# pswpswpsw/nif

Hardware: AMD Instinct MI355X
Metric: train-step points/sec (1D-wave, batch=1M per GPU) (higher is better)
Workload: dtype f32

## Files before the change

nif_amd/csrc/k_snet6.hip:

```cpp
#include "k_fuse_dev.h"

#define ZERO_T6(x) _Pragma("unroll") for (int b_ = 0; b_ < NBL; ++b_) { (x)[b_][0] = 0.f; (x)[b_][1] = 0.f; (x)[b_][2] = 0.f; (x)[b_][3] = 0.f; }

template <int NBL>
__device__ __forceinline__ void ring_store16(float* __restrict__ slot, const f32x4 (&h)[NBL], int g, int p) {
  float* q = slot + 4 * g * 16 + p;
#pragma unroll
  for (int b = 0; b < NBL; ++b)
#pragma unroll
    for (int v = 0; v < 4; ++v) q[(16 * b + v) * 16] = h[b][v];
}
template <int NBL>
__device__ __forceinline__ void ring_load16(const float* __restrict__ slot, f32x4 (&h)[NBL], int g, int p) {
  const float* q = slot + 4 * g * 16 + p;
#pragma unroll
  for (int b = 0; b < NBL; ++b)
#pragma unroll
    for (int v = 0; v < 4; ++v) h[b][v] = q[(16 * b + v) * 16];
}

#ifdef NIF_TIMELINE
#define S6_TL(id) do { if (blockIdx.x == 0 && (tid == 0 || tid == 512) && tlr == 2 && tlc < 380) { tlb[tlc] = ((long long)(id) << 48) | ((long long)__builtin_amdgcn_s_memtime() & 0xFFFFFFFFFFFFll); ++tlc; } } while (0)
#define S6_TL_FLUSH() do { if (A.tl && blockIdx.x == 0 && (tid == 0 || tid == 512)) for (int q_ = 0; q_ < tlc; ++q_) { A.tl[(tid ? 2048 : 0) + 2 * q_] = tlb[q_] >> 48; A.tl[(tid ? 2048 : 0) + 2 * q_ + 1] = tlb[q_] & 0xFFFFFFFFFFFFll; } } while (0)
#else
#define S6_TL(id) do { } while (0)
#define S6_TL_FLUSH() do { } while (0)
#endif
struct S6Args {
  SNetArgs s;
  float* partial; long pstride;
};

#ifndef NIF_S6_DBAR_T0
#define NIF_S6_DBAR_T0 5
#endif

constexpr int S6_WAVES = 8, S6_MAX_WG = 256;
constexpr int s6_ring(int NBL) { return 16 * NBL * 16; }

template <int NBL, int PR = 0>
__global__ __launch_bounds__(1024, 4) void k_snet6(S6Args F) {
  extern __shared__ __attribute__((aligned(256))) char smem6[];
  const SNetArgs& A = F.s;
  constexpr int NT = 512, WAVES = S6_WAVES, r = 1;
  constexpr int NCH = NBL / 2;
  constexpr bool X16 = PR == 0;
  constexpr int CF = X16 ? NBL * 2 * 64 : NBL * 3 * 64, CB = NBL * 2 * 64;
  constexpr bool CP = PR != 0;
  constexpr int CFH = CP ? NBL * 64 : CF, CBH = CP ? NBL * 64 : CB;
  constexpr PlaneSet HSET = CP ? PLANES_COMPACT : PLANES_HALF;
  static_assert(CFH == plane_chunk_units(HSET, PLANE_FWD, NBL) && CBH == plane_chunk_units(HSET, PLANE_BWD, NBL), "k_pack_dev.h");
  constexpr bool BIG = X16;
  constexpr int CFB = BIG ? 2 * CF : CF;
  constexpr int QF = (CFB + NT - 1) / NT;
  constexpr int NBUF = 2;
  constexpr int NPL = 6;
  constexpr int EXT = NPL * FUSE_PLANE_BYTES;
  constexpr int NVL = 5, NVF = 8, WVLT = NVL * 64, WVFT = NVF * 64;
  const int tid = threadIdx.x, wid = __builtin_amdgcn_readfirstlane(tid >> 6);
  const int lane = tid & 63, p = lane & 15, g = lane >> 4;
  const int n = A.n, nh = A.nh, si = A.si, so = A.so;
  const long nt16 = 2 * ((A.B + 31) / 32);
  const long ngroups = (nt16 + WAVES - 1) / WAVES;

  char* EX = smem6;
  char* WVL = EX + WAVES * EXT;
  char* WVF = WVL + WAVES * WVLT;
  bf16x8* chunks = reinterpret_cast<bf16x8*>(WVF + WAVES * WVFT);
  float* sm = reinterpret_cast<float*>(chunks + NBUF * CFB);
  constexpr int NP = 16 * NBL, RING = s6_ring(NBL);
  constexpr int o_w1 = 0, o_wl = 3 * NP, o_b1 = 6 * NP, o_bh = 7 * NP, o_bl = 11 * NP, nsm = 11 * NP + 4;
  constexpr int sm_tot = ((r + 1) * nsm + 3) & ~3;
  constexpr int CX = 3, CZ = 1, CY = 3;
  constexpr int NI = (CX + CZ + CY + 1) * 16;
  constexpr int pw = 2 * r * 64 + 2 * NI;
  float* lsum = sm + sm_tot + (long)WAVES * pw;
  float* scl = lsum + 16;
  long long* tlb = reinterpret_cast<long long*>(scl + 16) + (tid ? 380 : 0); (void)tlb;

  {
    const long s_wl = (long)si * n + (long)nh * n * n;
    const long s_b1 = s_wl + (long)n * so, s_bh = s_b1 + n, s_bl = s_bh + (long)nh * n;
    for (int idx = tid; idx < (r + 1) * nsm; idx += 1024) {
      const int k = idx / nsm, e = idx - k * nsm;
      float v = 0.f;
      if (e < o_wl) { const int dd = e / NP, f = e - dd * NP; if (f < n && dd < si) v = A.omega * hyp3(A, k, (long)dd * n + f); }
      else if (e < o_b1) { const int o = (e - o_wl) / NP, f = (e - o_wl) - o * NP; if (f < n && o < so) v = hyp3(A, k, s_wl + (long)f * so + o); }
      else if (e < o_bh) { const int f = e - o_b1; if (f < n) v = hyp3(A, k, s_b1 + f); }
      else if (e < o_bl) {
        const int j = (e - o_bh) / NP, f = (e - o_bh) - j * NP;
        if (f < n && j < nh) {
          v = hyp3(A, k, s_bh + (long)j * n + f);
          if (X16) v *= 4096.0f * A.wscale[(j * (r + 1) + k) * 2];
        }
      }
      else if (e < o_bl + so) v = hyp3(A, k, s_bl + (e - o_bl));
      sm[idx] = v;
    }
    if (X16 && tid < nh * (r + 1) * 2) scl[tid] = A.wscale[tid];
    for (int idx = tid; idx < (WAVES * (EXT + WVLT + WVFT)) / 16; idx += 1024) reinterpret_cast<f32x4*>(EX)[idx] = f32x4{0.f, 0.f, 0.f, 0.f};
  }

  const int NPC = (r + 1) * NCH;
  const bf16x8* cs_src = reinterpret_cast<const bf16x8*>(A.WF4);
  const int NPCS = BIG ? (r + 1) : NPC;
  int cs_units = BIG ? 2 * CFH : CFH, cs_left = nh * NPCS, cs_phase = 0;
  long cs_groups = (ngroups - 1 - (long)blockIdx.x) / gridDim.x;
  auto cs_phase_step = [&]() {
    ++cs_phase;
    if (cs_phase < 1 + nh) {
// ... 233 lines not shown
    return;
  }
#undef bacc
#undef facc
#undef fbacc
#undef lacc
#undef blacc

  float* dzs = sm + sm_tot + (long)wid * pw;
  float* sks = dzs + r * 64;
  float* inp = sks + r * 64;
  auto prefetch_inputs = [&](long tgn, int set) {
    long t16n = tgn * WAVES + wid;
    if (t16n >= nt16) t16n = nt16 - 1;
    const long tile32n = t16n >> 1;
    const int poffn = 16 * (int)(t16n & 1) + p;
    long ptn = t16n * 16 + p;
    if (ptn >= A.B) ptn = A.B - 1;
    float* dst = inp + set * NI;
    {
      const int c = g < si ? g : si - 1;
      const float* src = g < 3 ? A.xin + ptn * A.ncol + A.col0 + c : A.Z + (tile32n * r) * 32 + poffn;
      __builtin_amdgcn_global_load_lds((const __attribute__((address_space(1))) void*)src,
                                       (__attribute__((address_space(3))) void*)dst, 4, 0, 0);
    }
    {
      const int c = g < so ? g : so - 1;
      const float* src = (g < 3 || !A.sw) ? A.y + ptn * so + c : A.sw + ptn;
      __builtin_amdgcn_global_load_lds((const __attribute__((address_space(1))) void*)src,
                                       (__attribute__((address_space(3))) void*)(dst + 4 * 16), 4, 0, 0);
    }
  };
  prefetch_inputs(blockIdx.x, 0);
  if (cs_left <= 0) cs_left = -1;
  cs_next(0, true);
  __syncthreads();
  bool dma_mine = false;
  bool dma_early = false;
  int cbuf = 0, nbuf = 1;
  int tlc = 0, tlr = 0; (void)tlc; (void)tlr;
  float loss_lane = 0.f;
  float* ring = A.stash + ((long)blockIdx.x * WAVES + wid) * (long)nh * RING;
  const FuseDep dep = fuse_dep_addr(p, g);
  char* exw = EX + wid * EXT;

#define S6_CHUNK(...)                                                         \
  {                                                                           \
    S6_TL(100);                                                               \
    if (!dma_early) cs_next(nbuf, dma_mine);                                  \
    dma_early = false;                                                        \
    S6_TL(200);                                                               \
    const bf16x8* cur = chunks + cbuf * CFB;                                  \
    __VA_ARGS__                                                               \
    S6_TL(300);                                                               \
    __builtin_amdgcn_s_waitcnt(0x0070);         \
    S6_TL(400);                                                               \
    asm volatile("" ::: "memory");                                            \
    __builtin_amdgcn_s_barrier();                                             \
    asm volatile("" ::: "memory");                                            \
    S6_TL(500);                                                               \
    cbuf ^= 1; nbuf ^= 1;                                                     \
  }
#define S6_CHUNK2(ZI_, Q0_, Q1_, T_)                                          \
  S6_CHUNK({ mfma_x3<NBL, 3, ZI_, NBL, 0, false>(cur, Q0_[0], Q1_[0], T_, lane); mfma_x3<NBL, 3, false, NBL, 0, false>(cur + CF, Q0_[1], Q1_[1], T_, lane); })

  int iset = 0;
  for (long tg = blockIdx.x; tg < ngroups; tg += gridDim.x, ++iset, ++tlr) {
    S6_TL(1);
    const long t16_raw = tg * WAVES + wid;
    const bool active = t16_raw < nt16;
    const long t16 = active ? t16_raw : nt16 - 1;
    const long tile32 = t16 >> 1;
    const int poff = 16 * (int)(t16 & 1) + p;
    const long pt = t16 * 16 + p;
    const bool valid = active && pt < A.B;
    const float* xs = inp + (iset & 1) * NI + p;
    const float* zs = inp + (iset & 1) * NI + CX * 16;
    const float* ys = zs + CZ * 16 + p;
    const float* wsp = zs + (CZ + CY) * 16 + p;
    const float* zt_base = zs + p;
    dzs[lane] = 0.f;

    f32x4 h[NBL], acc[NBL];
    auto first_layer = [&](f32x4 (&out)[NBL]) __attribute__((always_inline)) {
      f32x4 a_[NBL];
      {
        const float* s0 = sm + r * nsm + 4 * g;
#pragma unroll
        for (int b = 0; b < NBL; ++b) {
          f32x4 s = *reinterpret_cast<const f32x4*>(s0 + o_b1 + 16 * b);
          _Pragma("unroll") for (int dd = 0; dd < 3; ++dd) if (dd < si) s += xs[dd * 16] * *reinterpret_cast<const f32x4*>(s0 + o_w1 + dd * NP + 16 * b);
          a_[b] = s;
        }
      }
      {
        const float zt = zt_base[0];
        const float* s0 = sm + 4 * g;
#pragma unroll
        for (int b = 0; b < NBL; ++b) {
          f32x4 s = *reinterpret_cast<const f32x4*>(s0 + o_b1 + 16 * b);
          _Pragma("unroll") for (int dd = 0; dd < 3; ++dd) if (dd < si) s += xs[dd * 16] * *reinterpret_cast<const f32x4*>(s0 + o_w1 + dd * NP + 16 * b);
          a_[b] += zt * s;
        }
      }
      sine16_tag<NBL>(a_, out);
    };
    first_layer(h);
    prefetch_inputs(tg + gridDim.x, (iset + 1) & 1);
    dma_mine = false;
    for (int j = 0; j < nh; ++j) {
      bf16x8 b0[NCH], b1[NCH], b2[NCH];
      if (X16) split2h<NBL>(h, 4096.0f, b0, b1);
      else split3p<NBL, PR>(h, b0, b1, b2);
      const float s1_ = X16 ? scl[j * 4 + 2] : 1.0f, is0_ = X16 ? scl[j * 4 + 1] : 1.0f, is1_ = X16 ? scl[j * 4 + 3] : 1.0f;
      {
        const float* sb = sm + r * nsm + o_bh + j * NP + 4 * g;
#pragma unroll
        for (int b = 0; b < NBL; ++b) acc[b] = *reinterpret_cast<const f32x4*>(sb + 16 * b);
      }
      {
        f32x4 T[NBL];
        const float* sb = sm + o_bh + j * NP + 4 * g;
#pragma unroll
        for (int b = 0; b < NBL; ++b) T[b] = *reinterpret_cast<const f32x4*>(sb + 16 * b);
#define S6_FWD(KS_, T_) mfma_x6<NBL, PR, false, NBL, 0, CP>(cur, b0[KS_], b1[KS_], b2[KS_], T_, lane);
        if (j > 0) ring_store16<NBL>(ring + j * RING, h, g, p);
        if (BIG) S6_CHUNK2(false, b0, b1, T)
        else {
          S6_CHUNK(S6_FWD(0, T))
          S6_CHUNK(S6_FWD(1, T))
        }
        const float zt = X16 ? zt_base[0] * (s1_ * is0_) : zt_base[0];
#pragma unroll
        for (int b = 0; b < NBL; ++b) acc[b] += zt * T[b];
      }
      if (BIG) S6_CHUNK2(false, b0, b1, acc)
      else {
        S6_CHUNK(S6_FWD(0, acc))
        S6_CHUNK(S6_FWD(1, acc))
      }
#undef S6_FWD
      if (X16) sine16_tag_sc<NBL>(acc, acc, is1_ * (1.0f / 4096.0f));
      else sine16_tag<NBL>(acc, acc);
#pragma unroll
      for (int b = 0; b < NBL; ++b) h[b] = acc[b];
    }
    f32x4 gh[NBL];
    ZERO_T6(gh)
    const float wsamp = (valid ? (A.sw ? wsp[0] : 1.0f) : 0.0f);
    const float zt0 = zt_base[0];
    float se = 0.f;
    for (int o = 0; o < so; ++o) {
      f32x4 wg[NBL];
      ZERO_T6(wg)
      float part = 0.f, bias = 0.f;
#pragma unroll
      for (int k = 0; k <= r; ++k) {
        const float zt = k < r ? zt0 : 1.0f;
        const float* s0 = sm + k * nsm;
        float sk = 0.f, sk2 = 0.f;
#pragma unroll
        for (int b = 0; b < NBL; ++b) {
          const f32x4 w = *reinterpret_cast<const f32x4*>(s0 + o_wl + o * NP + 16 * b + 4 * g);
          sk = fmaf(h[b][0], w[0], sk); sk2 = fmaf(h[b][1], w[1], sk2); sk = fmaf(h[b][2], w[2], sk); sk2 = fmaf(h[b][3], w[3], sk2);
          wg[b] += zt * w;
        }
        sk += sk2;
        part = fmaf(zt, sk, part);
        bias = fmaf(zt, s0[o_bl + o], bias);
        if (k < r) sks[k * 64 + lane] = sk;
      }
      part += __shfl_xor(part, 16);
      part += __shfl_xor(part, 32);
      const float uo = part + bias;
      const float e = uo - ys[o * 16];
      NIF_LOSS_ACC(A.loss_kind, e, se, dfac)
      const float du = dfac * wsamp * A.inv_bg / (float)so;
#pragma unroll
      for (int b = 0; b < NBL; ++b) gh[b] += du * wg[b];
      {
        float t = du * sks[lane];
        if (g == 0) t = fmaf(du, sm[o_bl + o], t);
        dzs[lane] += t;
      }
      if (g == 0 && o < 3) {
        __bf16* wv = reinterpret_cast<__bf16*>(WVL + wid * WVLT);
        const __bf16 d0 = (__bf16)du;
        wv[o * 32 + p] = d0; wv[o * 32 + 16 + p] = (__bf16)(du - (float)d0);
      }
    }
    if (g == 1) {
      __bf16* wv = reinterpret_cast<__bf16*>(WVL + wid * WVLT);
      const __bf16 z0 = (__bf16)zt0;
      wv[3 * 32 + p] = z0; wv[3 * 32 + 16 + p] = (__bf16)(zt0 - (float)z0);
    }
    {
      bf16x8 a0[NCH], a1[NCH];
      split2<NBL>(h, a0, a1);
      fuse_deposit4(exw, dep, a0);
      fuse_deposit4(exw + FUSE_PLANE_BYTES, dep, a1);
      f32x4 zh[NBL];
#pragma unroll
      for (int b = 0; b < NBL; ++b) zh[b] = zt0 * h[b];
      split2<NBL>(zh, a0, a1);
      fuse_deposit4(exw + 2 * FUSE_PLANE_BYTES, dep, a0);
      fuse_deposit4(exw + 3 * FUSE_PLANE_BYTES, dep, a1);
    }
    if (g == 0) loss_lane += wsamp * se / (float)so * A.inv_bg;
    if (BIG) {
      asm volatile("" ::: "memory");
      __builtin_amdgcn_s_waitcnt(0xC07F);
      S6_TL(600);
      __builtin_amdgcn_s_barrier();
      asm volatile("" ::: "memory");
      S6_TL(700);
    }
    f32x4 dnext[NBL], hin[NBL];
#pragma unroll
    for (int b = 0; b < NBL; ++b) hin[b] = h[b];
    dma_mine = true;
    for (int j = nh - 1; j >= 0; --j) {
      f32x4 ga[NBL];
      if (BIG) { cs_next(nbuf, true); dma_early = true; }
      tag_cos<NBL>(hin, dnext);
#pragma unroll
      for (int b = 0; b < NBL; ++b) ga[b] = dnext[b] * gh[b];
      {
        const float* sb = sm + o_bh + j * NP + 4 * g;
        float sbv = 0.f, sbv2 = 0.f;
#pragma unroll
        for (int b = 0; b < NBL; ++b) {
          const f32x4 bb = *reinterpret_cast<const f32x4*>(sb + 16 * b);
          sbv = fmaf(ga[b][0], bb[0], sbv); sbv2 = fmaf(ga[b][1], bb[1], sbv2); sbv = fmaf(ga[b][2], bb[2], sbv); sbv2 = fmaf(ga[b][3], bb[3], sbv2);
        }
        sbv += sbv2;
        dzs[lane] += X16 ? sbv * (scl[j * 4 + 1] * (1.0f / 4096.0f)) : sbv;
      }
      bf16x8 b0[NCH], b1[NCH];
      split2<NBL>(ga, b0, b1);
      bf16x8 q0[NCH], q1[NCH];
      const float s1_ = X16 ? scl[j * 4 + 2] : 1.0f, is0_ = X16 ? scl[j * 4 + 1] : 1.0f, is1_ = X16 ? scl[j * 4 + 3] : 1.0f;
      float ils = 1.0f;
      if (PR == 2 || X16) {
        float mx = 0.f;
#pragma unroll
        for (int b = 0; b < NBL; ++b) mx = fmaxf(fmaxf(mx, fmaxf(fabsf(ga[b][0]), fabsf(ga[b][1]))), fmaxf(fabsf(ga[b][2]), fabsf(ga[b][3])));
        mx = fmaxf(mx, __shfl_xor(mx, 16));
        mx = fmaxf(mx, __shfl_xor(mx, 32));
        const unsigned ef = (__float_as_uint(mx) >> 23) & 0xFFu;
        const unsigned sf = 268u - ef < 227u ? 268u - ef : 227u;
        ils = __uint_as_float((254u - sf) << 23);
        if (X16) split2h<NBL>(ga, __uint_as_float(sf << 23), q0, q1);
        else cast_f16<NBL>(ga, q0, __uint_as_float(sf << 23));
      } else {
#pragma unroll
        for (int ks = 0; ks < NCH; ++ks) q0[ks] = b0[ks];
      }
      if (!X16) {
#pragma unroll
        for (int ks = 0; ks < NCH; ++ks) q1[ks] = b1[ks];
      }
      {
        f32x4 U[NBL];
        if (j == 0) first_layer(hin); else ring_load16<NBL>(ring + j * RING, hin, g, p);
        if (BIG) S6_CHUNK2(true, q0, q1, U)
        else {
          S6_CHUNK({ mfma_x3<NBL, PR, true, NBL, 0, CP>(cur, q0[0], q1[0], U, lane); })
          S6_CHUNK({ mfma_x3<NBL, PR, false, NBL, 0, CP>(cur, q0[1], q1[1], U, lane); })
        }
        float s = 0.f;
#pragma unroll
        for (int b = 0; b < NBL; ++b)
#pragma unroll
          for (int v = 0; v < 4; ++v) s = fmaf(hin[b][v], U[b][v], s);
        const float ztc = X16 ? zt0 * (s1_ * is0_) : zt0;
#pragma unroll
        for (int b = 0; b < NBL; ++b) gh[b] = ztc * U[b];
        dzs[lane] += X16 ? (ils * is0_) * s : (PR == 2 ? ils * s : s);
      }
      if (BIG) S6_CHUNK2(false, q0, q1, gh)
      else {
        S6_CHUNK({ mfma_x3<NBL, PR, false, NBL, 0, CP>(cur, q0[0], q1[0], gh, lane); })
        S6_CHUNK({ mfma_x3<NBL, PR, false, NBL, 0, CP>(cur, q0[1], q1[1], gh, lane); })
      }
      if (PR == 2 || X16) {
        const float f_ = X16 ? ils * is1_ : ils;
#pragma unroll
        for (int b = 0; b < NBL; ++b) gh[b] *= f_;
      }
      {
        fuse_deposit4(exw + 4 * FUSE_PLANE_BYTES, dep, b0);
        fuse_deposit4(exw + 5 * FUSE_PLANE_BYTES, dep, b1);
        bf16x8 a0[NCH], a1[NCH];
        split2<NBL>(hin, a0, a1);
        fuse_deposit4(exw, dep, a0);
        fuse_deposit4(exw + FUSE_PLANE_BYTES, dep, a1);
        f32x4 zh[NBL];
#pragma unroll
        for (int b = 0; b < NBL; ++b) zh[b] = zt0 * hin[b];
        split2<NBL>(zh, a0, a1);
        fuse_deposit4(exw + 2 * FUSE_PLANE_BYTES, dep, a0);
        fuse_deposit4(exw + 3 * FUSE_PLANE_BYTES, dep, a1);
      }
      if (BIG && j > 0) {
        asm volatile("" ::: "memory");
        __builtin_amdgcn_s_waitcnt(0xC07F);
        S6_TL(600);
        __builtin_amdgcn_s_barrier();
        asm volatile("" ::: "memory");
        S6_TL(700);
      }
    }
    asm volatile("" ::: "memory");
    __builtin_amdgcn_s_waitcnt(0xC07F);
    __builtin_amdgcn_s_barrier();
    asm volatile("" ::: "memory");
    {
      f32x4 ga[NBL];
      tag_cos<NBL>(hin, dnext);
#pragma unroll
      for (int b = 0; b < NBL; ++b) ga[b] = dnext[b] * gh[b];
      {
        const float* s0 = sm + 4 * g;
        float s = 0.f, s2 = 0.f;
#pragma unroll
        for (int b = 0; b < NBL; ++b) {
          f32x4 t = *reinterpret_cast<const f32x4*>(s0 + o_b1 + 16 * b);
          _Pragma("unroll") for (int dd = 0; dd < 3; ++dd) if (dd < si) t += xs[dd * 16] * *reinterpret_cast<const f32x4*>(s0 + o_w1 + dd * NP + 16 * b);
          s = fmaf(ga[b][0], t[0], s); s2 = fmaf(ga[b][1], t[1], s2); s = fmaf(ga[b][2], t[2], s); s2 = fmaf(ga[b][3], t[3], s2);
        }
        float tot = dzs[lane] + (s + s2);
        tot += __shfl_xor(tot, 16);
        tot += __shfl_xor(tot, 32);
        if (active && g == 0) A.DZ[(tile32 * r) * 32 + poff] = tot;
      }
      bf16x8 b0[NCH], b1[NCH];
      split2<NBL>(ga, b0, b1);
      asm volatile("" ::: "memory");
      __builtin_amdgcn_s_waitcnt(0xC07F);
      __builtin_amdgcn_s_barrier();
      asm volatile("" ::: "memory");
      fuse_deposit4(exw + 4 * FUSE_PLANE_BYTES, dep, b0);
      fuse_deposit4(exw + 5 * FUSE_PLANE_BYTES, dep, b1);
      {
        __bf16* wv = reinterpret_cast<__bf16*>(WVF + wid * WVFT);
        const float x = g < si ? xs[g * 16] : 1.0f;
        const float zx = zt0 * x;
        const __bf16 x0 = (__bf16)x, z0 = (__bf16)zx;
        if (g < si || g == 3) { wv[g * 32 + p] = z0; wv[g * 32 + 16 + p] = (__bf16)(zx - (float)z0); }
        if (g < si && g < 3) { wv[(4 + g) * 32 + p] = x0; wv[(4 + g) * 32 + 16 + p] = (__bf16)(x - (float)x0); }
      }
    }
  }
#undef S6_CHUNK
  __syncthreads();
  __syncthreads();
  S6_TL_FLUSH();
  for (int off = 32; off > 0; off >>= 1) loss_lane += __shfl_down(loss_lane, off);
  if (lane == 0) lsum[wid] = loss_lane;
  __syncthreads();
  if (tid == 0) {
    float s = 0.f;
    for (int w = 0; w < WAVES; ++w) s += lsum[w];
    A.loss_partial[blockIdx.x] = s;
  }
}

static size_t snet6_shmem(const SNetArgs& a, int NBL) {
  const size_t sm_tot = (((size_t)(a.r + 1) * (11 * 16 * NBL + 4)) + 3) & ~(size_t)3;
  const size_t ni = 8 * 16;
  const size_t pw = 2 * a.r * 64 + 2 * ni;
  const size_t chunk = (size_t)(a.prec == 0 ? 2 : 1) * NBL * (a.prec == 0 ? 2 : 3) * 64 * 16;
  return 8 * (6 * FUSE_PLANE_BYTES + (5 + 8) * 64) + 2 * chunk + (sm_tot + 8 * pw + 16 + 16) * sizeof(float)
#ifdef NIF_TIMELINE
         + 2 * 380 * 8
#endif
      ;
}
bool snet6_supported(const SNetArgs& a) {
  if (a.ll || a.res || a.nif_skip) return false;
  if (a.prec != 0) {
    static const bool pol = [] { const char* e = getenv("NIF_S6_POLICY"); return !(e && e[0] == '0'); }();
    if (!pol) return false;
  }
  if (snet3_nbl(a.n) != 4 || a.r != 1 || a.nh < 1 || a.nh > 4 || a.si > 3 || a.so > 3) return false;
  if (a.prec == 0 && (!a.WF4x || !a.WB4x || !a.wscale)) return false;
  return snet6_shmem(a, 4) <= 160u * 1024u;
}
static long s6_workgroups(long B) {
  const long nt16 = 2 * ((B + 31) / 32);
  const long ngroups = (nt16 + S6_WAVES - 1) / S6_WAVES;
  return ngroups < S6_MAX_WG ? ngroups : S6_MAX_WG;
}
int snet6_rows(const SNetArgs& a) { return (int)s6_workgroups(a.B); }
long snet6_ring_floats(long B, int nh) { return s6_workgroups(B) * S6_WAVES * nh * s6_ring(4); }
int launch_snet6(const SNetArgs& a, float* partial, long pstride, hipStream_t st) {
  const int nblk = snet6_rows(a);
  S6Args f; f.s = a; f.partial = partial; f.pstride = pstride;
  const size_t shm = snet6_shmem(a, 4);
#define S6L(PR_)                                                                                                  \
  {                                                                                                               \
    (void)hipFuncSetAttribute((const void*)k_snet6<4, PR_>, hipFuncAttributeMaxDynamicSharedMemorySize, (int)shm); \
    hipLaunchKernelGGL((k_snet6<4, PR_>), dim3(nblk), dim3(1024), shm, st, f);                                    \
  }
  if (a.prec == 2) { f.s.WF4 = a.WF4h; f.s.WB4 = a.WB4h; S6L(2) }
  else if (a.prec == 1) { f.s.WF4 = a.WF4h; f.s.WB4 = a.WB4h; S6L(1) }
  else { f.s.WF4 = a.WF4x; f.s.WB4 = a.WB4x; S6L(0) }
#undef S6L
  return nblk;
}
```

nif_amd/csrc/nif_api.hip:

```cpp
#include "../../include/nif_hip.h"
#include "nif_internal.h"
#include "k_pack_dev.h"
#include <cstdlib>

#include <cmath>
#include <cstdio>
#include <cstring>
#include <memory>
#include <string>
#include <vector>

#include "nif_ctx.h"
#include "../../include/nif_hip_snapshots.h"
#include "../../include/nif_hip_encode.h"

#define NIF_ACT_SLABS 32
static inline bool act_on(const nif_ctx* c) { return c->act_l1 != 0.f || c->act_l2 != 0.f; }
struct RegsOff {
  nif_ctx* c; float jac_l1, act_l1, act_l2;
  RegsOff(nif_ctx* c_, bool on) : c(on ? c_ : nullptr) {
    if (!c) return;
    jac_l1 = c->jac_l1; act_l1 = c->act_l1; act_l2 = c->act_l2;
    c->jac_l1 = 0.f; c->act_l1 = 0.f; c->act_l2 = 0.f;
  }
// ... 1458 lines not shown
      launch_gw_out(g, c->NB, rows, c->st);
    }
    g = base; g.IN = c->use_wide ? nullptr : sST + (long)nms * c->slot_s; g.SM = c->DU; g.nc = c->so;
    g.W = dense_ref(0, 0, c->so); g.Bv = vec_ref(c->ll_bias, c->so);
    launch_gw_out(g, c->NB, rows, c->st);
    if (!fused_p) gw_pnet_stack(c, base, xin, c->stash_p, c->DZL, pa.omega, rows, c->st);
    g = base; g.IN = c->ZL; g.SM = c->DA; g.nc = c->r;
    g.W = dense_ref(c->last_w, c->r, c->r); g.Bv = vec_ref(c->last_b, c->r);
    launch_gw_out(g, c->RB, rows, c->st);
  }
  {
    ProfScope pr_(c, NIF_PROF_REDUCE);
    launch_reduce(c->partial, c->pstride, rows, c->loss_partial, nloss, c->grad, c->P, c->st);
  }
  if (n_act > 0) launch_add_sum(c->act_loss, n_act, c->grad + c->P, c->st);
  if (c->jac_l1 != 0.f) { int rc = jac_reg_pass(c, xin, B, Bg); if (rc) return rc; }
  if (nhead > 0) {
    { const int rca = ensure_jac_tmp(c); if (rca) return rca; }
    MuBlk mu;
    const long rr = (long)c->r * c->r;
    for (int e = 0; e < nhead; ++e) {
      mu.blk[sp->par[nsc + e]] = e;
      GwArgs g = gw_base(c, ntiles, B, c->partial);
      g.IN = c->ztl_par + (long)e * ntiles * 32 * 32 * c->RB; g.SM = c->dat_par + (long)e * ntiles * 32 * c->r; g.nc = c->r;
      g.W = dense_ref(c->last_w, c->r, c->r); g.Bv = vec_ref(c->last_b, c->r);
      launch_gw_out(g, c->RB, rows, c->st);
      launch_reduce(c->partial + c->last_w, c->pstride, rows, nullptr, 0, c->jac_tmp, rr, c->st);
      launch_axpy_cols(c->grad + c->last_w, c->jac_tmp, rr, c->P - c->last_w, c->st);
    }
    HIPCHK(hipGetLastError());
    return jac_reg_pass(c, xin, B, Bg, mu.blk);
  }
  HIPCHK(hipGetLastError());
  return NIF_OK;
}

static int snet_plan(nif_ctx* c, SNetArgs& sa, int ns, const int* seeds, int* nloss, const SobPlan* sp = nullptr) {
  int rc;
  if (ns > 0) {
    SobPar spq{};
    if (sp) spq = sob_par_of(*sp);
    const int nblk = launch_sob(sa, true, ns, seeds, nullptr, 0.f, nullptr, nullptr, true, c->st, sp ? &spq : nullptr);
    if (nblk < 0)
      return fail(NIF_ERR_INVALID, "Sobolev step: the kernel's working set of this shape (units, latent_dim, parameter columns) does not fit the 160 KB LDS of a CU");
    const long need = (long)nblk * 4 * sob_ring_floats_per_wave(c->n, c->nh);
    rc = c->dring.reserve(c, need); if (rc) return rc;
    *nloss = nblk;
  } else if (c->use_snet3 || c->use_snet4) {
    int waves = 4;
    const int nblk = c->use_snet4 ? launch_snet4(sa, true, true, c->st) : launch_snet3(sa, true, true, &waves, c->st);
    const long need = (long)nblk * waves * snet3_ring_floats_per_wave(c->n, c->nh);
    rc = c->dring.reserve(c, need); if (rc) return rc;
    *nloss = nblk;
  }
  sa.dring = c->dring;
  return NIF_OK;
}

static long pipe_chunk_points(const nif_ctx* c, long B) {
  long ch = c->opt_pipe_chunk;
  if (ch < 0) ch = 0;
  if (ch <= 0) return 0;
  ch = (ch + 2047) / 2048 * 2048;
  return ch;
}

static int ensure_pipe(nif_ctx* c, int nchunk) {
  if (!c->st2) {
    HIPCHK(hipStreamCreateWithFlags(&c->st2, hipStreamNonBlocking));
    HIPCHK(hipEventCreateWithFlags(&c->ev_start, hipEventDisableTiming));
    HIPCHK(hipEventCreateWithFlags(&c->ev_done, hipEventDisableTiming));
  }
  while ((int)c->ev_chunk.size() < nchunk) {
    hipEvent_t e;
    HIPCHK(hipEventCreateWithFlags(&e, hipEventDisableTiming));
    c->ev_chunk.push_back(e);
  }
  return c->chunk_grad.reserve(c, (long)nchunk * c->pstride);
}

static int step_chunk(nif_ctx* c, const float* xin0, const float* y0, const float* sw0, long off, long B, long Bg, int ns,
                      const int* seeds, const float* gt, float wj, hipStream_t sa_st, hipStream_t sb_st, hipStream_t pb_st,
                      float* partial, float* loss_partial, int* nloss_out, int chunk_idx, bool whole, SNetArgs* sa_out = nullptr,
                      const SobPlan* sp = nullptr) {
  int rc;
  const int ncol = c->pi + c->si;
  const long ntiles = (B + 31) / 32, t0 = off / 32;
  const float* xin = xin0 + off * ncol;
  const float* y = y0 + off * c->so;
  const float* sw = sw0 ? sw0 + off : nullptr;
  PNetArgs pa; fill_pnet(c, pa, xin, B);
  pa.Z = c->Z + t0 * 32 * c->r; pa.DZ = c->DZ + t0 * 32 * c->r;
  if (pa.stash) pa.stash += t0 * 32 * 32 * c->NSTB;
  const bool fused_p = !pnet_force_stash() && pnet_bwg_supported(pa);
  if (!fused_p) { const int rcp = ensure_packed_p32(c); if (rcp) return rcp; }
  { ProfScope p_(c, NIF_PROF_PNET_FWD, sa_st); launch_pnet(pa, c->NSTB, !fused_p, sa_st); }
  SNetArgs sa; fill_snet(c, sa, xin, ncol, c->pi, B);
  sa.Z = pa.Z; sa.DZ = pa.DZ; sa.DU = c->DU + t0 * 32 * c->so;
  sa.stash = c->stash_s + t0 * 32 * 32 * c->NB;
  sa.y = y; sa.sw = sw; sa.u_out = nullptr; sa.loss_partial = loss_partial; sa.inv_bg = 1.0f / (float)Bg;
  if (!whole) sa.wg_cap = c->opt_pipe_wgs;
  int nloss = (int)((ntiles + 3) / 4);
  rc = snet_plan(c, sa, ns, seeds, &nloss, sp); if (rc) return rc;
  const bool fused_gw = ns == 0 && whole && c->use_snet4 && c->opt_fuse_gw && snet6_supported(sa) &&
                        snet6_rows(sa) == rows_for(c, ntiles);
  if (fused_gw) nloss = snet6_rows(sa);
  *nloss_out = nloss;
  {
    const int nbl = snet3_nbl(c->n);
    bool dab = sa.prec == 1 && (nbl == 2 || nbl == 4 || nbl == 8) && gw_da_bf16_ok(c->NB, c->NB, c->r);
    if (ns > 0) dab = dab && sobw_supported(sa, ns, sp && sp->any_par);
    else dab = dab && c->use_snet4 && !fused_gw;
    sa.da_bf16 = dab ? 1 : 0;
    sa.h_ph16 = (dab && ns == 0 && nbl == 8 && !c->cfg.s_resblock && !sa.nif_skip && gw_in_ph16_ok(c->NB, c->NB, c->r)) ? 1 : 0;
  }
  const bool wrote_da_bf16 = ns > 0 ? sob_writes_da_bf16(sa, ns, sp && sp->any_par)
                                    : (!fused_gw && c->use_snet4 && snet4_writes_da_bf16(sa));
  if (wrote_da_bf16 != (sa.da_bf16 != 0)) return fail(NIF_ERR_STATE, "internal: dL/da stash format of producer and plan disagree");
  const bool wrote_h_ph16 = ns == 0 && !fused_gw && c->use_snet4 && snet4_writes_h_ph16(sa);
  if (wrote_h_ph16 != (sa.h_ph16 != 0)) return fail(NIF_ERR_STATE, "internal: layer-input stash format of producer and plan disagree");
  {
    ProfScope p_(c, NIF_PROF_SNET, sa_st);
    if (ns > 0) {
      SobPar spar{};
      if (sp) spar = sob_par_of(*sp);
      if (sp && sp->any_par) { spar.ZT = c->zt_par; spar.DZT = c->dzt_par; }
      launch_sob(sa, true, ns, seeds, gt, wj, c->dring, nullptr, false, sa_st, sp ? &spar : nullptr);
    }
    else if (fused_gw) launch_snet6(sa, partial, c->pstride, sa_st);
    else if (c->use_snet4) { if (launch_snet4(sa, true, false, sa_st) < 0) return fail(NIF_ERR_STATE, "internal: no k_snet4 form for this net (SIREN planes not packed as half pairs)"); }
    else if (c->use_snet3) launch_snet3(sa, true, false, nullptr, sa_st);
    else launch_snet(sa, c->NB, true, sa_st);
  }
  if (act_on(c)) {
    const long nlp = (B + 255) / 256;
    rc = c->act_loss.reserve(c, nlp); if (rc) return rc;
    const bool l1 = c->act_l2 == 0.f;
    launch_actreg_points(l1, c->theta, c->last_w, c->last_b, c->r, c->po, sa.Z, B, (l1 ? c->act_l1 : c->act_l2) / (float)Bg, sa.DZ,
                         c->act_loss, sa_st);
  }
  if (sb_st != sa_st || pb_st != sa_st) {
    HIPCHK(hipEventRecord(c->ev_chunk[chunk_idx], sa_st));
    if (sb_st != sa_st) HIPCHK(hipStreamWaitEvent(sb_st, c->ev_chunk[chunk_idx], 0));
    if (pb_st != sa_st && pb_st != sb_st) HIPCHK(hipStreamWaitEvent(pb_st, c->ev_chunk[chunk_idx], 0));
  }
  const int rows = rows_for(c, ntiles);
  { ProfScope p_(c, NIF_PROF_PNET_BWD, pb_st);
    static const bool touch_on = [] { const char* e = getenv("NIF_PBW_TOUCH"); return !(e && e[0] == '0'); }();
    const float* touch = (touch_on && whole && pb_st == sb_st && !fused_gw) ? sa.stash + (long)(c->nh + 1) * c->slot_s : nullptr;
    if (fused_p) launch_pnet_bwg(pa, partial, c->pstride, rows, pb_st, touch, (long)c->NB * 1024);
    else launch_pnet_bwd(pa, c->NSTB, pb_st); }
  ProfScope pgw(c, NIF_PROF_GW, sb_st);
  const GwArgs base = gw_base(c, ntiles, B, partial);
  if (!fused_gw) {
    GwArgs sbase = base;
    gw_add_tangents(sbase, ns, seeds);
    long first_ntiles = sbase.ntiles;
    if (sp) first_ntiles = ntiles * (1 + sp->nsc);
    if (sp && sp->hess) first_ntiles = ntiles * 3;
    if (gw_hyper_snet_stack(c, sbase, sa, xin, sa.Z, 0, first_ntiles, wrote_da_bf16, wrote_h_ph16, rows, sb_st) < 0)
      return fail(NIF_ERR_STATE, "internal: bf16 dL/da stash rows without a reader of that form");
  }
  if (!fused_p) gw_pnet_stack(c, base, xin, pa.stash, pa.DZ, pa.omega, rows, pb_st);
  if (sa_out) *sa_out = sa;
  HIPCHK(hipGetLastError());
  return NIF_OK;
}

static int ensure_small_tables(nif_ctx* c, const PNetArgs& pa, const SNetArgs& sa) {
  if (c->small_idx) return NIF_OK;
  if (c->capturing) return fail(NIF_ERR_STATE, "small-batch step tables inside a graph capture (nif_graph_begin builds them)");
  std::vector<int> idx, desc;
  small_tables(pa, sa, idx, desc);
  DevBuf<int> d_idx, d_desc;
  int rc = d_idx.alloc((long)idx.size()); if (rc) return rc;
  rc = d_desc.alloc((long)desc.size()); if (rc) return rc;
  HIPCHK(hipMemcpy(d_idx, idx.data(), idx.size() * sizeof(int), hipMemcpyHostToDevice));
  HIPCHK(hipMemcpy(d_desc, desc.data(), desc.size() * sizeof(int), hipMemcpyHostToDevice));
  c->small_idx = std::move(d_idx); c->small_desc = std::move(d_desc);
  return NIF_OK;
}
int nif_tail_flush(nif_ctx* c) {
  if (!c->tail_pending) return NIF_OK;
  c->tail_pending = false;
  launch_reduce(c->partial, c->pstride, c->tail_rows, c->loss_partial, c->tail_nloss, c->grad, c->P, c->st);
  HIPCHK(hipGetLastError());
  return NIF_OK;
}
static bool tail_can_defer(const nif_ctx* c) {
  if (!c->opt_fuse_tail || c->comm || c->capturing || c->prof_on) return false;
  if ((c->reg_l1 != 0.f || c->reg_l2 != 0.f) && c->reg_hi > c->reg_lo) return false;
  if (c->sreg_l1 != 0.f || c->sreg_l2 != 0.f) return false;
  return true;
}
int nif_metric_flush(nif_ctx* c) {
  if (!c->metric_pending) return NIF_OK;
  const int rc = nif_tail_flush(c); if (rc) return rc;
  c->metric_pending = false;
  launch_metric(c->grad, c->P, c->metric_pending_w, c->metric, c->st);
  HIPCHK(hipGetLastError());
  return NIF_OK;
}
int nif_enter(nif_ctx* c, nif_flush what) {
  HIPCHK(hipSetDevice(c->dev));
  if (what == NIF_FLUSH_NONE) return NIF_OK;
  const int rc = nif_tail_flush(c); if (rc) return rc;
  return what == NIF_FLUSH_METRIC ? nif_metric_flush(c) : NIF_OK;
}
static int loss_grad_core(nif_ctx* c, const float* xin, const float* y, const float* sw, int64_t B, int64_t Bg, int ns,
                          const int* seeds, const float* gt, float wj, const SobPlan* sp = nullptr) {
  c->last_step_small = false;
  if (ns == 0 && c->opt_small_step && B <= NIF_SMALL_MAX_B && c->kind != NIF_KIND_LASTLAYER && !act_on(c) && !c->opt_fp32_mfma) {
    if (!c->have_params) return fail(NIF_ERR_STATE, "parameters not set (call nif_set_params first)");
    PNetArgs pa; fill_pnet(c, pa, xin, B);
    SNetArgs sa; fill_snet(c, sa, xin, c->pi + c->si, c->pi, B);
    if (small_supported(pa, sa) && small_rows(B) <= 256) {
      int rc = ensure_rows(c, B); if (rc) return rc;
      const int rows = small_rows(B);
      if (rows > c->rows_cap()) return fail(NIF_ERR_STATE, "internal: partial-row buffer too small for the small-batch step");
      if (rows > c->loss_partial.n) return fail(NIF_ERR_STATE, "internal: loss partial buffer too small for the small-batch step");
      c->grad_rewritten();
      sa.y = y; sa.sw = sw; sa.loss_partial = c->loss_partial; sa.inv_bg = 1.0f / (float)Bg;
      rc = ensure_small_tables(c, pa, sa); if (rc) return rc;
      const bool mp = c->metric_pending && c->metric != nullptr;
      { ProfScope p_(c, NIF_PROF_SNET);
        launch_small(pa, sa, c->partial, c->pstride, c->P, c->small_idx, c->small_desc, mp ? c->metric : nullptr, c->metric_pending_w,
                     c->grad + c->P, c->st); }
      if (mp) c->metric_pending = false;
      c->last_step_small = true;
      if (c->jac_l1 == 0.f && tail_can_defer(c)) { c->tail_pending = true; c->tail_rows = rows; c->tail_nloss = rows; }
      else { ProfScope pr_(c, NIF_PROF_REDUCE); launch_reduce(c->partial, c->pstride, rows, c->loss_partial, rows, c->grad, c->P, c->st); }
      if (c->jac_l1 != 0.f) { rc = jac_reg_pass(c, xin, B, Bg); if (rc) return rc; }
      HIPCHK(hipGetLastError());
      return NIF_OK;
    }
  }
  int rc = nif_metric_flush(c); if (rc) return rc;
  rc = ensure_packed(c); if (rc) return rc;
  const long ntiles = (B + 31) / 32;
  if (ns > 0) { rc = ensure_packed32(c); if (rc) return rc; }
  if (ns > 0) {
    if (c->kind != NIF_KIND_LASTLAYER && !c->jac_ok)
      return fail(NIF_ERR_INVALID, "Sobolev training: one weight plane and the small hyper-vectors of this shape exceed the 160 KB LDS of a CU");
    if (c->cfg.s_resblock && (c->nh & 1)) return fail(NIF_ERR_INVALID, "resblock ShapeNet with an odd matrix count");
  }
  rc = ensure_capacity(c, ntiles * 32 * (1 + ns), true); if (rc) return rc;
  if (sp && sp->any_par) {
    PNetArgs pa; fill_pnet(c, pa, xin, B);
    rc = ensure_zt_par(c, pa, ntiles, true); if (rc) return rc;
  }
  c->grad_rewritten();
  if (c->kind == NIF_KIND_LASTLAYER) return loss_grad_ll(c, xin, y, sw, B, Bg, ns, sp, gt, wj);
  const long chunk = (ns == 0 && c->use_snet3 && !act_on(c) && c->jac_l1 == 0.f) ? pipe_chunk_points(c, B) : 0;
  if (chunk <= 0 || chunk >= B) {
    int nloss = 0;
    SNetArgs sae;
    const bool side = c->opt_side_pnet && B >= 65536;
    if (side) { rc = ensure_pipe(c, 1); if (rc) return rc; }
    rc = step_chunk(c, xin, y, sw, 0, B, Bg, ns, seeds, gt, wj, c->st, c->st, side ? c->st2 : c->st, c->partial, c->loss_partial,
                    &nloss, 0, true, &sae, sp);
    if (rc) return rc;
    if (side) {
      HIPCHK(hipEventRecord(c->ev_done, c->st2));
      HIPCHK(hipStreamWaitEvent(c->st, c->ev_done, 0));
    }
    const int rows = rows_for(c, ntiles);
    if (ns == 0 && !act_on(c) && c->jac_l1 == 0.f && !(sp && sp->any_par) && tail_can_defer(c)) {
      c->tail_pending = true; c->tail_rows = rows; c->tail_nloss = nloss;
      HIPCHK(hipGetLastError());
      return NIF_OK;
    }
    ProfScope pr_(c, NIF_PROF_REDUCE);
    launch_reduce(c->partial, c->pstride, rows, c->loss_partial, nloss, c->grad, c->P, c->st);
    if (act_on(c)) {
      const long need = (long)NIF_ACT_SLABS * (c->r + 1) * c->po;
      rc = c->act_part.reserve(c, need); if (rc) return rc;
      const bool l1 = c->act_l2 == 0.f;
      launch_actreg_planes(l1, c->theta, c->last_w, c->last_b, c->r, c->po, c->Z, B, NIF_ACT_SLABS, c->act_part, c->st);
      launch_actreg_apply(c->act_part, NIF_ACT_SLABS, c->r, c->po, (l1 ? c->act_l1 : c->act_l2) / (float)Bg, c->last_w, c->last_b,
                          c->act_loss, (int)((B + 255) / 256), c->grad, c->P, c->st);
    }
    if (c->jac_l1 != 0.f) { rc = jac_reg_pass(c, xin, B, Bg); if (rc) return rc; }
    if (sp && sp->any_par) { rc = sob_par_pass(c, xin, B, Bg, *sp, sae); if (rc) return rc; }
    HIPCHK(hipGetLastError());
    return NIF_OK;
  }
  const int nchunk = (int)((B + chunk - 1) / chunk);
  rc = ensure_pipe(c, nchunk); if (rc) return rc;
  HIPCHK(hipEventRecord(c->ev_start, c->st));
  HIPCHK(hipStreamWaitEvent(c->st2, c->ev_start, 0));
  const long lp_stride = c->loss_partial.n / nchunk;
  for (int i = 0; i < nchunk; ++i) {
    const long off = (long)i * chunk;
    const long Bc = B - off < chunk ? B - off : chunk;
    int nloss = 0;
    rc = step_chunk(c, xin, y, sw, off, Bc, Bg, 0, nullptr, nullptr, 0.f, c->st, c->st2, c->st2, c->partial,
                    c->loss_partial + i * lp_stride, &nloss, i, false);
    if (rc) return rc;
    if (nloss > lp_stride) return fail(NIF_ERR_STATE, "loss partial buffer too small for the chunk pipeline");
    const int rows = rows_for(c, (Bc + 31) / 32);
    launch_reduce(c->partial, c->pstride, rows, c->loss_partial + i * lp_stride, nloss, c->chunk_grad + (long)i * c->pstride, c->P, c->st2);
  }
  HIPCHK(hipEventRecord(c->ev_done, c->st2));
  HIPCHK(hipStreamWaitEvent(c->st, c->ev_done, 0));
  {
    ProfScope pr_(c, NIF_PROF_REDUCE);
    launch_reduce(c->chunk_grad, c->pstride, nchunk, nullptr, 0, c->grad, c->P + 1, c->st);
  }
  HIPCHK(hipGetLastError());
  return NIF_OK;
}

extern "C" int nif_loss_grad_dev(nif_ctx* c, const float* xin, const float* y, const float* sw, int64_t B, int64_t Bg) {
  if (!c || !xin || !y || B <= 0 || Bg < B) return fail(NIF_ERR_INVALID, "bad argument");
  NIF_ENTER(c, NIF_FLUSH_TAIL)
  return loss_grad_core(c, xin, y, sw, B, Bg, 0, nullptr, nullptr, 0.f);
}

extern "C" int nif_reserve(nif_ctx* c, int64_t B_max, int32_t n_tangents) {
  if (!c || B_max <= 0 || n_tangents < 0 || n_tangents > 16) return fail(NIF_ERR_INVALID, "bad argument");
  if (n_tangents > 3) n_tangents = 3;
  NIF_ENTER(c, NIF_FLUSH_TAIL)
  int rc = ensure_packed(c); if (rc) return rc;
  const long ntiles = (B_max + 31) / 32;
  rc = ensure_capacity(c, ntiles * 32 * (1 + n_tangents), true); if (rc) return rc;
  if (c->kind == NIF_KIND_LASTLAYER) {
    if (c->use_ll4) {
      SNetArgs sa; fill_snet_ll(c, sa, nullptr, c->pi + c->si, c->pi, B_max);
      int nblk = 0;
      rc = ll4_plan(c, sa, &nblk); if (rc) return rc;
    }
    return NIF_OK;
  }
  SNetArgs sa; fill_snet(c, sa, nullptr, c->pi + c->si, c->pi, B_max);
  int nloss = 0;
  const int seeds[3] = {0, 0, 0};
  rc = snet_plan(c, sa, n_tangents, seeds, &nloss); if (rc) return rc;
  const long chunk = (n_tangents == 0 && c->use_snet3) ? pipe_chunk_points(c, B_max) : 0;
  if (chunk > 0 && chunk < B_max) { rc = ensure_pipe(c, (int)((B_max + chunk - 1) / chunk)); if (rc) return rc; }
  return NIF_OK;
}

static int sobolev_plan(nif_ctx* c, const int32_t* x_idx, int32_t nx, SobPlan* sp) {
  if (!x_idx || nx < 1 || nx > 3) return fail(NIF_ERR_INVALID, "internal: a Sobolev pass carries 1..3 columns");
  memset(sp, 0, sizeof(*sp));
// ... 924 lines not shown
```

Baseline: 942.7 million.

## Use sqrt-based cosine, permlane swaps, rolled first-layer loop, and same-stream pnet for fused path

Replaces the cosine derivative with sqrt(1-sin^2) plus a sign bit copied from the stored sine. Cross-group reductions now use permlane16/32 swap builtins instead of xor shuffles. The first-layer evaluation is shared through a helper with a non-unrolled input loop, so the backward recompute reuses it. When the fused gradient-weight kernel runs, the parameter-net backward is kept on the main stream instead of a side stream, which drops the event sync. The sqrt form is accurate only when the stored tag sign matches the cosine sign, and the rolled loop may add loop overhead.

```diff
diff --git a/nif_amd/csrc/k_snet6.hip b/nif_amd/csrc/k_snet6.hip
--- a/nif_amd/csrc/k_snet6.hip
+++ b/nif_amd/csrc/k_snet6.hip
@@ -1,4 +1,5 @@
 #include "k_fuse_dev.h"
+#include <type_traits>
 
 #define ZERO_T6(x) _Pragma("unroll") for (int b_ = 0; b_ < NBL; ++b_) { (x)[b_][0] = 0.f; (x)[b_][1] = 0.f; (x)[b_][2] = 0.f; (x)[b_][3] = 0.f; }
 
@@ -26,6 +27,33 @@
 #define S6_TL(id) do { } while (0)
 #define S6_TL_FLUSH() do { } while (0)
 #endif
+typedef unsigned u32x4 __attribute__((ext_vector_type(4)));
+template <int NBL>
+__device__ __forceinline__ void tag_cos4(const f32x4 (&sn)[NBL], f32x4 (&d)[NBL]) {
+#pragma unroll
+  for (int b = 0; b < NBL; ++b) {
+    f32x4 c;
+#pragma unroll
+    for (int v = 0; v < 4; ++v) {
+      const float s = sn[b][v];
+      c[v] = __builtin_amdgcn_sqrtf(__builtin_amdgcn_fmed3f(fmaf(-s, s, 1.0f), 0.0f, 1.0f));
+    }
+    d[b] = __builtin_bit_cast(f32x4, __builtin_bit_cast(u32x4, c) | (__builtin_bit_cast(u32x4, sn[b]) << 31));
+  }
+}
+__device__ __forceinline__ float s6_sum_groups(float x) {
+  auto q = __builtin_amdgcn_permlane16_swap(__float_as_uint(x), __float_as_uint(x), false, false);
+  x = __uint_as_float(q[0]) + __uint_as_float(q[1]);
+  q = __builtin_amdgcn_permlane32_swap(__float_as_uint(x), __float_as_uint(x), false, false);
+  return __uint_as_float(q[0]) + __uint_as_float(q[1]);
+}
+__device__ __forceinline__ float s6_max_groups(float x) {
+  auto q = __builtin_amdgcn_permlane16_swap(__float_as_uint(x), __float_as_uint(x), false, false);
+  x = fmaxf(__uint_as_float(q[0]), __uint_as_float(q[1]));
+  q = __builtin_amdgcn_permlane32_swap(__float_as_uint(x), __float_as_uint(x), false, false);
+  return fmaxf(__uint_as_float(q[0]), __uint_as_float(q[1]));
+}
+
 struct S6Args {
   SNetArgs s;
   float* partial; long pstride;
@@ -425,27 +453,31 @@
     dzs[lane] = 0.f;
 
     f32x4 h[NBL], acc[NBL];
+    auto first_rows = [&](f32x4 (&a_)[NBL], f32x4 (&s_)[NBL], auto both) __attribute__((always_inline)) {
+      constexpr bool BOTH = decltype(both)::value;
+      const float* s1 = sm + r * nsm + 4 * g;
+      const float* s0 = sm + 4 * g;
+#pragma unroll
+      for (int b = 0; b < NBL; ++b) {
+        if (BOTH) a_[b] = *reinterpret_cast<const f32x4*>(s1 + o_b1 + 16 * b);
+        s_[b] = *reinterpret_cast<const f32x4*>(s0 + o_b1 + 16 * b);
+      }
+#pragma clang loop unroll(disable)
+      for (int dd = 0; dd < si; ++dd) {
+        const float x = xs[dd * 16];
+#pragma unroll
+        for (int b = 0; b < NBL; ++b) {
+          if (BOTH) a_[b] += x * *reinterpret_cast<const f32x4*>(s1 + o_w1 + dd * NP + 16 * b);
+          s_[b] += x * *reinterpret_cast<const f32x4*>(s0 + o_w1 + dd * NP + 16 * b);
+        }
+      }
+    };
     auto first_layer = [&](f32x4 (&out)[NBL]) __attribute__((always_inline)) {
-      f32x4 a_[NBL];
-      {
-        const float* s0 = sm + r * nsm + 4 * g;
-#pragma unroll
-        for (int b = 0; b < NBL; ++b) {
-          f32x4 s = *reinterpret_cast<const f32x4*>(s0 + o_b1 + 16 * b);
-          _Pragma("unroll") for (int dd = 0; dd < 3; ++dd) if (dd < si) s += xs[dd * 16] * *reinterpret_cast<const f32x4*>(s0 + o_w1 + dd * NP + 16 * b);
-          a_[b] = s;
-        }
-      }
-      {
-        const float zt = zt_base[0];
-        const float* s0 = sm + 4 * g;
-#pragma unroll
-        for (int b = 0; b < NBL; ++b) {
-          f32x4 s = *reinterpret_cast<const f32x4*>(s0 + o_b1 + 16 * b);
-          _Pragma("unroll") for (int dd = 0; dd < 3; ++dd) if (dd < si) s += xs[dd * 16] * *reinterpret_cast<const f32x4*>(s0 + o_w1 + dd * NP + 16 * b);
-          a_[b] += zt * s;
-        }
-      }
+      f32x4 a_[NBL], s_[NBL];
+      first_rows(a_, s_, std::true_type{});
+      const float zt = zt_base[0];
+#pragma unroll
+      for (int b = 0; b < NBL; ++b) a_[b] += zt * s_[b];
       sine16_tag<NBL>(a_, out);
     };
     first_layer(h);
@@ -513,8 +545,7 @@
         bias = fmaf(zt, s0[o_bl + o], bias);
         if (k < r) sks[k * 64 + lane] = sk;
       }
-      part += __shfl_xor(part, 16);
-      part += __shfl_xor(part, 32);
+      part = s6_sum_groups(part);
       const float uo = part + bias;
       const float e = uo - ys[o * 16];
       NIF_LOSS_ACC(A.loss_kind, e, se, dfac)
@@ -565,7 +596,7 @@
     for (int j = nh - 1; j >= 0; --j) {
       f32x4 ga[NBL];
       if (BIG) { cs_next(nbuf, true); dma_early = true; }
-      tag_cos<NBL>(hin, dnext);
+      tag_cos4<NBL>(hin, dnext);
 #pragma unroll
       for (int b = 0; b < NBL; ++b) ga[b] = dnext[b] * gh[b];
       {
@@ -588,8 +619,7 @@
         float mx = 0.f;
 #pragma unroll
         for (int b = 0; b < NBL; ++b) mx = fmaxf(fmaxf(mx, fmaxf(fabsf(ga[b][0]), fabsf(ga[b][1]))), fmaxf(fabsf(ga[b][2]), fabsf(ga[b][3])));
-        mx = fmaxf(mx, __shfl_xor(mx, 16));
-        mx = fmaxf(mx, __shfl_xor(mx, 32));
+        mx = s6_max_groups(mx);
         const unsigned ef = (__float_as_uint(mx) >> 23) & 0xFFu;
         const unsigned sf = 268u - ef < 227u ? 268u - ef : 227u;
         ils = __uint_as_float((254u - sf) << 23);
@@ -660,21 +690,19 @@
     asm volatile("" ::: "memory");
     {
       f32x4 ga[NBL];
-      tag_cos<NBL>(hin, dnext);
+      tag_cos4<NBL>(hin, dnext);
 #pragma unroll
       for (int b = 0; b < NBL; ++b) ga[b] = dnext[b] * gh[b];
       {
-        const float* s0 = sm + 4 * g;
+        f32x4 t[NBL];
+        first_rows(t, t, std::false_type{});
         float s = 0.f, s2 = 0.f;
 #pragma unroll
         for (int b = 0; b < NBL; ++b) {
-          f32x4 t = *reinterpret_cast<const f32x4*>(s0 + o_b1 + 16 * b);
-          _Pragma("unroll") for (int dd = 0; dd < 3; ++dd) if (dd < si) t += xs[dd * 16] * *reinterpret_cast<const f32x4*>(s0 + o_w1 + dd * NP + 16 * b);
-          s = fmaf(ga[b][0], t[0], s); s2 = fmaf(ga[b][1], t[1], s2); s = fmaf(ga[b][2], t[2], s); s2 = fmaf(ga[b][3], t[3], s2);
+          s = fmaf(ga[b][0], t[b][0], s); s2 = fmaf(ga[b][1], t[b][1], s2); s = fmaf(ga[b][2], t[b][2], s); s2 = fmaf(ga[b][3], t[b][3], s2);
         }
         float tot = dzs[lane] + (s + s2);
-        tot += __shfl_xor(tot, 16);
-        tot += __shfl_xor(tot, 32);
+        tot = s6_sum_groups(tot);
         if (active && g == 0) A.DZ[(tile32 * r) * 32 + poff] = tot;
       }
       bf16x8 b0[NCH], b1[NCH];
diff --git a/nif_amd/csrc/nif_api.hip b/nif_amd/csrc/nif_api.hip
--- a/nif_amd/csrc/nif_api.hip
+++ b/nif_amd/csrc/nif_api.hip
@@ -1564,7 +1564,7 @@
 static int step_chunk(nif_ctx* c, const float* xin0, const float* y0, const float* sw0, long off, long B, long Bg, int ns,
                       const int* seeds, const float* gt, float wj, hipStream_t sa_st, hipStream_t sb_st, hipStream_t pb_st,
                       float* partial, float* loss_partial, int* nloss_out, int chunk_idx, bool whole, SNetArgs* sa_out = nullptr,
-                      const SobPlan* sp = nullptr) {
+                      const SobPlan* sp = nullptr, bool* pb_aside = nullptr) {
   int rc;
   const int ncol = c->pi + c->si;
   const long ntiles = (B + 31) / 32, t0 = off / 32;
@@ -1588,6 +1588,8 @@
                         snet6_rows(sa) == rows_for(c, ntiles);
   if (fused_gw) nloss = snet6_rows(sa);
   *nloss_out = nloss;
+  if (fused_gw) pb_st = sb_st;
+  if (pb_aside) *pb_aside = pb_st != sa_st;
   {
     const int nbl = snet3_nbl(c->n);
     bool dab = sa.prec == 1 && (nbl == 2 || nbl == 4 || nbl == 8) && gw_da_bf16_ok(c->NB, c->NB, c->r);
@@ -1739,10 +1741,11 @@
     SNetArgs sae;
     const bool side = c->opt_side_pnet && B >= 65536;
     if (side) { rc = ensure_pipe(c, 1); if (rc) return rc; }
+    bool aside = false;
     rc = step_chunk(c, xin, y, sw, 0, B, Bg, ns, seeds, gt, wj, c->st, c->st, side ? c->st2 : c->st, c->partial, c->loss_partial,
-                    &nloss, 0, true, &sae, sp);
+                    &nloss, 0, true, &sae, sp, &aside);
     if (rc) return rc;
-    if (side) {
+    if (aside) {
       HIPCHK(hipEventRecord(c->ev_done, c->st2));
       HIPCHK(hipStreamWaitEvent(c->st, c->ev_done, 0));
     }
```

Result: faster. 952.6 million (median of 6 runs) (+1.0%).
